# jaxsonpd/air_rs

Measured on AMD Instinct MI355X. Metric: IQ Msamples/s (decoded Mode-S msgs/s alongside), 2 MSPS i8 stream, higher is better.
Workload: dtype i8; 1 GPU; 2 MSPS i8 IQ, 1 GiB synthetic buffer per GPU, fused magnitude+preamble/DF17 gate+PPM+CRC-24; samples_per_gpu=536870912, bytes_per_gpu=1073741824, channels=1

## Files before the change

### air_rs_amd/csrc/adsb_kernels.hip

```cpp
#include <hip/hip_ext.h>
#include <utility>
#include <cstdlib>

#include "adsb_kernels.h"
#include "adsb_synth.h"

namespace adsbk {

typedef unsigned int u32x4 __attribute__((ext_vector_type(4)));
typedef unsigned short u16x2 __attribute__((ext_vector_type(2)));

__device__ __forceinline__ uint32_t pkmin(uint32_t a, uint32_t b)
{
    u16x2 r = __builtin_elementwise_min(__builtin_bit_cast(u16x2, a), __builtin_bit_cast(u16x2, b));
    return __builtin_bit_cast(uint32_t, r);
}
__device__ __forceinline__ uint32_t pkmax(uint32_t a, uint32_t b)
{
    u16x2 r = __builtin_elementwise_max(__builtin_bit_cast(u16x2, a), __builtin_bit_cast(u16x2, b));
    return __builtin_bit_cast(uint32_t, r);
}
typedef _Float16 f16x2 __attribute__((ext_vector_type(2)));
template <bool F16> __device__ __forceinline__ uint32_t pkmax3(uint32_t a, uint32_t b, uint32_t c)
{
    if (F16) {
        f16x2 r = __builtin_elementwise_maximum(
            __builtin_elementwise_maximum(__builtin_bit_cast(f16x2, a), __builtin_bit_cast(f16x2, b)),
            __builtin_bit_cast(f16x2, c));
        return __builtin_bit_cast(uint32_t, r);
    }
    return pkmax(pkmax(a, b), c);
}
template <bool F16> __device__ __forceinline__ uint32_t pkmin3(uint32_t a, uint32_t b, uint32_t c)
{
    if (F16) {
        f16x2 r = __builtin_elementwise_minimum(
            __builtin_elementwise_minimum(__builtin_bit_cast(f16x2, a), __builtin_bit_cast(f16x2, b)),
            __builtin_bit_cast(f16x2, c));
        return __builtin_bit_cast(uint32_t, r);
    }
    return pkmin(pkmin(a, b), c);
}

__device__ __forceinline__ void dot4x8_sacc(u32x4 v, int c, int n[8])
{
    const uint32_t a0 = v.x & 0xFFFFu, a1 = v.x & 0xFFFF0000u, a2 = v.y & 0xFFFFu, a3 = v.y & 0xFFFF0000u,
                   a4 = v.z & 0xFFFFu, a5 = v.z & 0xFFFF0000u, a6 = v.w & 0xFFFFu, a7 = v.w & 0xFFFF0000u;
    asm("v_dot4_i32_i8 %0, %8, %12, %20\n\t"
        "v_dot4_i32_i8 %1, %8, %13, %20\n\t"
        "v_dot4_i32_i8 %2, %9, %14, %20\n\t"
        "v_dot4_i32_i8 %3, %9, %15, %20\n\t"
        "v_dot4_i32_i8 %4, %10, %16, %20\n\t"
        "v_dot4_i32_i8 %5, %10, %17, %20\n\t"
        "v_dot4_i32_i8 %6, %11, %18, %20\n\t"
        "v_dot4_i32_i8 %7, %11, %19, %20\n\t"
        "s_nop 2"
        : "=&v"(n[0]), "=&v"(n[1]), "=&v"(n[2]), "=&v"(n[3]), "=&v"(n[4]), "=&v"(n[5]), "=&v"(n[6]), "=&v"(n[7])
        : "v"(v.x), "v"(v.y), "v"(v.z), "v"(v.w), "v"(a0), "v"(a1), "v"(a2), "v"(a3), "v"(a4), "v"(a5),
          "v"(a6), "v"(a7), "s"(c));
}

struct SynTable {
    uint32_t v[112];
};
constexpr SynTable make_syn()
{
    SynTable t{};
    uint32_t r = 1;
    for (int e = 0; e < 112; ++e) {
        t.v[111 - e] = r;
        r <<= 1;
        if (r & 0x1000000u) r ^= 0x1FFF409u;
    }
    return t;
}
__constant__ SynTable kSyn = make_syn();

template <int MAGMODE> __device__ __forceinline__ float mag_root_i8(int n_plus_2p23)
{
    float f = __builtin_bit_cast(float, n_plus_2p23) - 8388607.5f;
    float r = __builtin_amdgcn_sqrtf(f);
    if (MAGMODE == 2) r -= 0.5f;
    return r;
}

typedef float f32x2 __attribute__((ext_vector_type(2)));
template <int MAGMODE>
__device__ __forceinline__ void mags8_i8(u32x4 v, uint32_t &lo, uint32_t &hi)
{
    int n[8];
    dot4x8_sacc(v, 0x4B000000, n);
    float f[8];
#pragma unroll
    for (int k = 0; k < 8; k += 2) {
        f32x2 t = {__builtin_bit_cast(float, n[k]), __builtin_bit_cast(float, n[k + 1])};
        t = t - (f32x2){8388607.5f, 8388607.5f};
        f[k] = t.x;
        f[k + 1] = t.y;
    }
    float r[8];
#pragma unroll
    for (int k = 0; k < 8; ++k) {
        r[k] = __builtin_amdgcn_sqrtf(f[k]);
        if (MAGMODE == 2) r[k] -= 0.5f;
    }
    lo = __builtin_amdgcn_cvt_pk_u8_f32(r[0], 0, 0u);
    lo = __builtin_amdgcn_cvt_pk_u8_f32(r[1], 1, lo);
    lo = __builtin_amdgcn_cvt_pk_u8_f32(r[2], 2, lo);
    lo = __builtin_amdgcn_cvt_pk_u8_f32(r[3], 3, lo);
    hi = __builtin_amdgcn_cvt_pk_u8_f32(r[4], 0, 0u);
    hi = __builtin_amdgcn_cvt_pk_u8_f32(r[5], 1, hi);
    hi = __builtin_amdgcn_cvt_pk_u8_f32(r[6], 2, hi);
    hi = __builtin_amdgcn_cvt_pk_u8_f32(r[7], 3, hi);
}

__device__ __forceinline__ uint32_t mag_i16_fix(uint32_t r, uint32_t n)
{
    return r - ((__umul24(r, r) > n) ? 1u : 0u);
}
__device__ __forceinline__ uint32_t mag_i16(uint32_t iq)
{
    uint32_t n, r;
    asm("v_dot2_i32_i16 %0, %2, %2, 0\n\t"
        "s_nop 2\n\t"
        "v_cvt_f32_u32 %1, %0\n\t"
        "v_sqrt_f32 %1, %1\n\t"
        "s_nop 0\n\t"
        "v_cvt_rpi_i32_f32 %1, %1"
        : "=&v"(n), "=&v"(r)
        : "v"(iq));
    return mag_i16_fix(r, n);
}
__device__ __forceinline__ void mags4_i16(u32x4 v, uint32_t &lo, uint32_t &hi)
{
    uint32_t n0, n1, n2, n3, r0, r1, r2, r3;
    asm("v_dot2_i32_i16 %0, %8, %8, 0\n\t"
        "v_dot2_i32_i16 %1, %9, %9, 0\n\t"
        "v_dot2_i32_i16 %2, %10, %10, 0\n\t"
        "v_dot2_i32_i16 %3, %11, %11, 0\n\t"
        "s_nop 2\n\t"
        "v_cvt_f32_u32 %4, %0\n\t"
        "v_cvt_f32_u32 %5, %1\n\t"
        "v_cvt_f32_u32 %6, %2\n\t"
        "v_cvt_f32_u32 %7, %3\n\t"
        "v_sqrt_f32 %4, %4\n\t"
        "v_sqrt_f32 %5, %5\n\t"
        "v_sqrt_f32 %6, %6\n\t"
        "v_sqrt_f32 %7, %7\n\t"
        "v_cvt_rpi_i32_f32 %4, %4\n\t"
        "v_cvt_rpi_i32_f32 %5, %5\n\t"
        "v_cvt_rpi_i32_f32 %6, %6\n\t"
        "s_nop 0\n\t"
        "v_cvt_rpi_i32_f32 %7, %7\n\t"
        "s_nop 0"
        : "=&v"(n0), "=&v"(n1), "=&v"(n2), "=&v"(n3), "=&v"(r0), "=&v"(r1), "=&v"(r2), "=&v"(r3)
        : "v"(v.x), "v"(v.y), "v"(v.z), "v"(v.w));
    lo = __builtin_amdgcn_perm(mag_i16_fix(r1, n1), mag_i16_fix(r0, n0), 0x05040100u);
    hi = __builtin_amdgcn_perm(mag_i16_fix(r3, n3), mag_i16_fix(r2, n2), 0x05040100u);
}

__global__ void probe_cvt_kernel(uint32_t *out)
{
// ... 139 lines not shown
            "v_cmp_gt_u32_sdwa %7, %12, %12 src0_sel:BYTE_0 src1_sel:BYTE_1\n\t"
            "v_cmp_gt_u32_sdwa %8, %12, %12 src0_sel:BYTE_2 src1_sel:BYTE_3\n\t"
            "v_addc_co_u32_e64 %0, vcc, %0, %0, %1\n\t"
            "v_addc_co_u32_e64 %0, vcc, %0, %0, %2\n\t"
            "v_addc_co_u32_e64 %0, vcc, %0, %0, %3\n\t"
            "v_addc_co_u32_e64 %0, vcc, %0, %0, %4\n\t"
            "v_addc_co_u32_e64 %0, vcc, %0, %0, %5\n\t"
            "v_addc_co_u32_e64 %0, vcc, %0, %0, %6\n\t"
            "v_addc_co_u32_e64 %0, vcc, %0, %0, %7\n\t"
            "v_addc_co_u32_e64 %0, vcc, %0, %0, %8"
            : "+v"(byte), "=&s"(m0), "=&s"(m1), "=&s"(m2), "=&s"(m3), "=&s"(m4), "=&s"(m5), "=&s"(m6), "=&s"(m7)
            : "v"(w[0]), "v"(w[1]), "v"(w[2]), "v"(w[3])
            : "vcc");
    }
    return byte;
}

__device__ __forceinline__ uint32_t nsq_slice_byte(const uint32_t *img, const uint32_t off, const uint32_t l)
{
    const uint32_t half = off >= (uint32_t)kNsqHalf ? 1u : 0u;
    const uint32_t base = off - half * (uint32_t)kNsqHalf + 16u;
    const uint32_t e = base & 15u, par = e & 1u, sh = e >> 1;
    const uint32_t v = (base >> 4) + l;
    const uint32_t a1 = nsq_phys(16u * v) + par;
    constexpr uint32_t kChunksPerBlock = (1u << kNsqPadShift) / 16u;
    const uint32_t a2 = a1 + 15u + (((v & (kChunksPerBlock - 1u)) == kChunksPerBlock - 1u ? 4u : 0u) & (0u - par));
    uint32_t d[16];
#pragma unroll
    for (int j = 0; j < 15; ++j) d[j] = img[a1 + j];
    d[15] = img[a2];
    const uint32_t sel = half ? 0x07060302u : 0x05040100u;
    uint32_t w[8], r2[8];
#pragma unroll
    for (int j = 0; j < 8; ++j) {
        w[j] = __builtin_amdgcn_perm(d[2 * j + 1], d[2 * j], sel);
        const float fx = (float)(w[j] & 0xFFFFu) - ((float)kNsqBias - 0.5f);
        const uint32_t r = (uint32_t)__builtin_amdgcn_sqrtf(fx);
        r2[j] = __umul24(r, r) + (uint32_t)kNsqBias;
    }
    uint32_t chunk = 0;
    uint64_t m0, m1, m2, m3, m4, m5, m6, m7;
    asm("v_cmp_gt_u32_sdwa %1, %9, %17 src0_sel:DWORD src1_sel:WORD_1\n\t"
        "v_cmp_gt_u32_sdwa %2, %10, %18 src0_sel:DWORD src1_sel:WORD_1\n\t"
        "v_cmp_gt_u32_sdwa %3, %11, %19 src0_sel:DWORD src1_sel:WORD_1\n\t"
        "v_cmp_gt_u32_sdwa %4, %12, %20 src0_sel:DWORD src1_sel:WORD_1\n\t"
        "v_cmp_gt_u32_sdwa %5, %13, %21 src0_sel:DWORD src1_sel:WORD_1\n\t"
        "v_cmp_gt_u32_sdwa %6, %14, %22 src0_sel:DWORD src1_sel:WORD_1\n\t"
        "v_cmp_gt_u32_sdwa %7, %15, %23 src0_sel:DWORD src1_sel:WORD_1\n\t"
        "v_cmp_gt_u32_sdwa %8, %16, %24 src0_sel:DWORD src1_sel:WORD_1\n\t"
        "v_addc_co_u32_e64 %0, vcc, %0, %0, %1\n\t"
        "v_addc_co_u32_e64 %0, vcc, %0, %0, %2\n\t"
        "v_addc_co_u32_e64 %0, vcc, %0, %0, %3\n\t"
        "v_addc_co_u32_e64 %0, vcc, %0, %0, %4\n\t"
        "v_addc_co_u32_e64 %0, vcc, %0, %0, %5\n\t"
        "v_addc_co_u32_e64 %0, vcc, %0, %0, %6\n\t"
        "v_addc_co_u32_e64 %0, vcc, %0, %0, %7\n\t"
        "v_addc_co_u32_e64 %0, vcc, %0, %0, %8"
        : "+v"(chunk), "=&s"(m0), "=&s"(m1), "=&s"(m2), "=&s"(m3), "=&s"(m4), "=&s"(m5), "=&s"(m6), "=&s"(m7)
        : "v"(r2[0]), "v"(r2[1]), "v"(r2[2]), "v"(r2[3]), "v"(r2[4]), "v"(r2[5]), "v"(r2[6]), "v"(r2[7]),
          "v"(w[0]), "v"(w[1]), "v"(w[2]), "v"(w[3]), "v"(w[4]), "v"(w[5]), "v"(w[6]), "v"(w[7])
        : "vcc");
    const uint32_t next = (uint32_t)__builtin_amdgcn_update_dpp(0, (int)chunk, 0x101 , 0xF, 0xF, true);
    return (((chunk << 8) | next) >> (8u - sh)) & 0xFFu;
}

__device__ __forceinline__ bool count_candidate(const bool have, const uint32_t byte, const uint32_t l, const uint32_t lane)
{
    const uint32_t lb = l < 14 ? l : 13;
    uint32_t s = 0;
    const uint32_t *sy = kSyn.v + 8 * lb;
    const int sb = (int)(l < 14 ? byte : 0u);
#pragma unroll
    for (int k = 0; k < 8; ++k) s ^= sy[k] & (uint32_t)((sb << (24 + k)) >> 31);
    s = row16_xor(s);
    int found = -1;
    if (s != 0 && l < 11) {
#pragma unroll
        for (int k = 0; k < 8; ++k) found = (sy[k] == s) ? k : found;
    }
    const unsigned long long fm = __ballot(found >= 0);
    const uint32_t gbits = (uint32_t)(fm >> (lane & 48u)) & 0xFFFFu;
    return have && (s == 0 || gbits != 0);
}

struct TilePos {
    uint32_t ch;
    uint64_t sample0;
    uint32_t n_valid;
};
template <int TILE = kTile>
__device__ __forceinline__ TilePos tile_pos(const DemodArgs &p, uint32_t tile)
{
    TilePos t;
    t.ch = tile / p.tiles_per_channel;
    const uint32_t tch = tile - t.ch * p.tiles_per_channel;
    t.sample0 = (uint64_t)tch * TILE;
    const uint64_t left = (p.n_samples - kWindow) - t.sample0;
    t.n_valid = left < (uint64_t)TILE ? (uint32_t)left : (uint32_t)TILE;
    return t;
}

template <int BPS, int MAG = kMag>
__device__ __forceinline__ __amdgpu_buffer_rsrc_t tile_rsrc(const DemodArgs &p, const TilePos &t, bool live = true)
{
    const char *base = (const char *)p.iq + ((uint64_t)t.ch * p.channel_stride + t.sample0) * BPS;
    const uint64_t remain = (p.n_samples - t.sample0) * BPS;
    const uint32_t nrec = remain > (uint64_t)(MAG * BPS) ? (uint32_t)(MAG * BPS) : (uint32_t)remain;
    return __builtin_amdgcn_make_buffer_rsrc((void *)base, 0, live ? (int)nrec : 0, 0x00020000);
}

#ifndef ADSB_TILE_STAMPS
#define ADSB_TILE_STAMPS 0
#endif
#if ADSB_TILE_STAMPS
#define TSTAMP(k)                                                                                              \
    do {                                                                                                       \
        if ((tid & 63u) == 0 && (wave == 0 || wave == 3)) {                                                    \
            __builtin_amdgcn_sched_barrier(0);                                                                 \
            const unsigned long long now_ = __builtin_amdgcn_s_memtime();                                      \
            if ((k) >= 0) ts_seg[(k)] = (uint32_t)(now_ - ts_prev);                                            \
            ts_prev = now_;                                                                                    \
            __builtin_amdgcn_sched_barrier(0);                                                                 \
        }                                                                                                      \
    } while (0)
#else
#define TSTAMP(k) do { } while (0)
#endif

#ifndef ADSB_ABL_PHASES
#define ADSB_ABL_PHASES 3
#endif
#ifndef ADSB_ABL_NOCMP
#define ADSB_ABL_NOCMP 0
#endif
#ifndef ADSB_AB_KERNELS
#define ADSB_AB_KERNELS 0
#endif
bool ab_kernels_built() { return ADSB_AB_KERNELS != 0; }
#ifndef ADSB_PRIO
#define ADSB_PRIO 0
#endif
#ifndef ADSB_GATE_GROUP
#define ADSB_GATE_GROUP 1
#endif

template <int RUN, int NT>
__device__ __forceinline__ void gate_collect(uint32_t *candA, uint32_t *candB, uint16_t *list, uint32_t *count,
                                             const uint32_t tid, const uint32_t n_valid)
{
    constexpr int WPR = (RUN + 31) / 32;
    const uint32_t sa = tid * RUN, sb = (tid + NT) * RUN;
    const uint32_t va = n_valid > sa ? (n_valid - sa) : 0u, vb = n_valid > sb ? (n_valid - sb) : 0u;
    uint32_t words[2 * WPR];
    uint32_t nz = 0, c = 0;
#pragma unroll
    for (int k = 0; k < WPR; ++k) {
        words[k] = candA[k];
        words[WPR + k] = candB[k];
    }
    if (n_valid < (uint32_t)(2 * NT * RUN)) {
#pragma unroll
        for (int k = 0; k < WPR; ++k) {
            const uint32_t la = va > 32u * k ? va - 32u * k : 0u, lb = vb > 32u * k ? vb - 32u * k : 0u;
            words[k] &= la >= 32u ? 0xFFFFFFFFu : ((1u << la) - 1u);
            words[WPR + k] &= lb >= 32u ? 0xFFFFFFFFu : ((1u << lb) - 1u);
            candA[k] = words[k];
            candB[k] = words[WPR + k];
        }
    }
#pragma unroll
    for (int k = 0; k < 2 * WPR; ++k) {
        nz |= words[k];
        c += __builtin_popcount(words[k]);
    }
    if (nz) {
        uint32_t pos = atomicAdd(count, c);
#pragma unroll
        for (int k = 0; k < 2 * WPR; ++k) {
            uint32_t bits = words[k];
            const uint32_t base = (k < WPR ? sa : sb) + (k % WPR) * 32;
            while (bits) {
                const uint32_t b = __builtin_ctz(bits);
                bits &= bits - 1;
                if (pos < (uint32_t)kSparseCap) list[pos] = (uint16_t)(base + b);
                ++pos;
            }
        }
    }
}

struct NoHook {
    __device__ __forceinline__ void operator()() const {}
};

template <int ST, int GROUP, int RUN, int NT, int HOOK_AT = -1, class HOOK = NoHook, bool F16OK = (ST == ADSB_SAMPLE_I8), bool PAD = false>
__device__ __forceinline__ void gate_phase(const typename MagT<ST>::type *mag, uint32_t *cand, uint16_t *list,
                                           uint32_t *count, const uint32_t tid, const uint32_t n_valid,
                                           HOOK hook = HOOK())
{
    static_assert(RUN % GROUP == 0 && (RUN == 16 || RUN == 32 || RUN == 64), "steps are taken GROUP at a time; 1 or 2 bitmap words per run");
    constexpr int WPR = (RUN + 31) / 32;
    constexpr int SPG = 16 / (int)sizeof(typename MagT<ST>::type);
    uint32_t *candA = cand + WPR * tid, *candB = cand + WPR * (tid + NT);
#pragma unroll
    for (int k = 0; k < WPR; ++k) candA[k] = candB[k] = 0u;
    constexpr int kGran = (RUN + 26 + SPG - 1) / SPG + 1;
    static_assert(!PAD || (ST == ADSB_SAMPLE_I8 && RUN == 32 && (NT * RUN) % 256 == 0), "the padded image: u8 magnitudes, runs of 32 bytes");
    const u32x4 *ga = reinterpret_cast<const u32x4 *>(mag + mag_phys<PAD>(tid * RUN));
    const u32x4 *gb = reinterpret_cast<const u32x4 *>(mag + mag_phys<PAD>((tid + NT) * RUN));
    const uint32_t hop = PAD && (tid & 7u) == 7u ? 1u : 0u;
    const u32x4 *ga2 = ga + hop, *gb2 = gb + hop;
    uint32_t ra[kGran * 4], rb[kGran * 4];
    constexpr int kAhead = 48 / SPG;
#pragma unroll
    for (int g = 0; g < kAhead; ++g) {
        u32x4 a = (PAD && g >= 2) ? ga2[g] : ga[g], b = (PAD && g >= 2) ? gb2[g] : gb[g];
        ra[4 * g] = a.x; ra[4 * g + 1] = a.y; ra[4 * g + 2] = a.z; ra[4 * g + 3] = a.w;
        rb[4 * g] = b.x; rb[4 * g + 1] = b.y; rb[4 * g + 2] = b.z; rb[4 * g + 3] = b.w;
    }

    uint32_t N[RUN + 26], H2[RUN + 8], W3[RUN + 16], F[RUN + 9];
#pragma unroll
    for (int k = 0; k < 25; ++k) N[k] = pair_at<ST>(ra, rb, k);
#pragma unroll
    for (int j = 0; j < 7; ++j) H2[j] = pkmin(N[j], N[j + 2]);
#pragma unroll
    for (int j = 3; j < 13; ++j) W3[j] = pkmax3<F16OK>(N[j], N[j + 1], N[j + 2]);
#pragma unroll
    for (int j = 1; j < 8; ++j) F[j] = pkmax3<F16OK>(N[j], W3[j + 2], N[j + 5]);

#if ADSB_ABL_NOCMP
    uint32_t abl_acc = 0;
#endif
#pragma unroll
    for (int o0 = 0; o0 < RUN; o0 += GROUP) {
        if (o0 == HOOK_AT) hook();
        bool pa[GROUP], pb[GROUP];
        bool any = false;
#pragma unroll
        for (int gi = 0; gi < GROUP; ++gi) {
            const int o = o0 + gi;
            if (o % SPG == 0) {
                const int g = o / SPG + kAhead;
                if (g * SPG < RUN + 26) {
                    u32x4 a = (PAD && g >= 2) ? ga2[g] : ga[g], b = (PAD && g >= 2) ? gb2[g] : gb[g];
                    ra[4 * g] = a.x; ra[4 * g + 1] = a.y; ra[4 * g + 2] = a.z; ra[4 * g + 3] = a.w;
                    rb[4 * g] = b.x; rb[4 * g + 1] = b.y; rb[4 * g + 2] = b.z; rb[4 * g + 3] = b.w;
                }
            }
            N[o + 25] = pair_at<ST>(ra, rb, o + 25);
            W3[o + 13] = pkmax3<F16OK>(N[o + 13], N[o + 14], N[o + 15]);
            F[o + 8] = pkmax3<F16OK>(N[o + 8], W3[o + 10], N[o + 13]);
            const uint32_t lo = pkmax3<F16OK>(F[o + 1], F[o + 8], W3[o + 13]);
            H2[o + 7] = pkmin(N[o + 7], N[o + 9]);
            const uint32_t hi = pkmin(H2[o], H2[o + 7]);
#if ADSB_ABL_NOCMP
            abl_acc ^= hi ^ lo;
            pa[gi] = pb[gi] = false;
#else
            pa[gi] = (uint16_t)hi >= (uint16_t)lo;
            pb[gi] = (hi >> 16) >= (lo >> 16);
            any |= pa[gi] | pb[gi];
#endif
        }
        if (__builtin_expect(__builtin_amdgcn_ballot_w64(any) != 0, 0)) {
#pragma unroll
            for (int gi = 0; gi < GROUP; ++gi) {
                const int o = o0 + gi;
                if (GROUP == 1 || __builtin_amdgcn_ballot_w64(pa[gi] | pb[gi]) != 0) {
                    const uint32_t dh = pkmin3<F16OK>(pkmin3<F16OK>(N[o + 16], N[o + 19], N[o + 21]), N[o + 23], N[o + 24]);
                    const uint32_t dl = pkmax3<F16OK>(pkmax3<F16OK>(N[o + 17], N[o + 18], N[o + 20]), N[o + 22], N[o + 25]);
                    const bool da = (uint16_t)dh >= (uint16_t)dl;
                    const bool db = (dh >> 16) >= (dl >> 16);
                    uint32_t bit = 1u << (o & 31);
                    asm("" : "+v"(bit));
                    if (pa[gi] & da) atomicOr(candA + (o >> 5), bit);
                    if (pb[gi] & db) atomicOr(candB + (o >> 5), bit);
                }
            }
        }
    }
#if ADSB_ABL_NOCMP
    if (abl_acc == 0x12345678u) atomicOr(candA, 1u);
#endif
    gate_collect<RUN, NT>(candA, candB, list, count, tid, n_valid);
}

template <int BPS, int MAG = kMag>
__device__ __forceinline__ u32x4 tile_rsrc_words(const DemodArgs &p, const TilePos &t, bool live)
{
    const uint64_t base = (uint64_t)(uintptr_t)((const char *)p.iq + ((uint64_t)t.ch * p.channel_stride + t.sample0) * BPS);
    const uint64_t remain = (p.n_samples - t.sample0) * BPS;
    const uint32_t nrec = remain > (uint64_t)(MAG * BPS) ? (uint32_t)(MAG * BPS) : (uint32_t)remain;
    u32x4 w;
    w.x = __builtin_amdgcn_readfirstlane((uint32_t)base);
    w.y = __builtin_amdgcn_readfirstlane((uint32_t)(base >> 32) & 0xFFFFu);
    w.z = __builtin_amdgcn_readfirstlane(live ? nrec : 0u);
    w.w = 0x00020000u;
    return w;
}

#ifndef ADSB_LOAD_AUX
#define ADSB_LOAD_AUX 2
#endif
template <int ST> struct P1 {
    static constexpr int kSPL = ST == ADSB_SAMPLE_I8 ? 8 : 4;
    static constexpr int kIters = (TileCfg<ST>::kMagT + kThreads * kSPL - 1) / (kThreads * kSPL);
};

template <int ST>
__device__ __forceinline__ void issue_tile_loads(const DemodArgs &p, const TilePos &tp, bool live, uint32_t tid,
                                                 u32x4 (&raw)[P1<ST>::kIters])
{
    constexpr int BPS = (ST == ADSB_SAMPLE_I8) ? 2 : 4;
    __amdgpu_buffer_rsrc_t rsrc = tile_rsrc<BPS, TileCfg<ST>::kMagT>(p, tp, live);
    const uint32_t wave_s0 = __builtin_amdgcn_readfirstlane(tid & ~63u) * P1<ST>::kSPL;
#pragma unroll
    for (int it = 0; it < P1<ST>::kIters; ++it)
        if ((uint32_t)it * (kThreads * P1<ST>::kSPL) + wave_s0 < (uint32_t)TileCfg<ST>::kMagT)
            raw[it] = __builtin_amdgcn_raw_buffer_load_b128(rsrc, tid * 16, (uint32_t)it * (kThreads * 16), ADSB_LOAD_AUX);
}

template <int ST, int MAGMODE, bool PAD = false>
__device__ __forceinline__ bool magnitudes_to_lds(const u32x4 (&raw)[P1<ST>::kIters], typename MagT<ST>::type *mag, uint32_t tid)
{
    uint32_t mx = 0;
    const uint32_t wave_s0 = __builtin_amdgcn_readfirstlane(tid & ~63u) * P1<ST>::kSPL;
#pragma unroll
    for (int it = 0; it < P1<ST>::kIters; ++it) {
        if ((uint32_t)it * (kThreads * P1<ST>::kSPL) + wave_s0 < (uint32_t)TileCfg<ST>::kMagT) {
            const uint32_t s = (uint32_t)it * (kThreads * P1<ST>::kSPL) + tid * P1<ST>::kSPL;
            uint32_t lo, hi;
            if (ST == ADSB_SAMPLE_I8) mags8_i8<MAGMODE>(raw[it], lo, hi);
            else {
                mags4_i16(raw[it], lo, hi);
                mx = pkmax(mx, pkmax(lo, hi));
            }
            const uint32_t sp = PAD ? s + 16u * (tid >> 5) + (uint32_t)it * (16u * (kThreads * P1<ST>::kSPL / 256)) : s;
            if (s < (uint32_t)TileCfg<ST>::kMagT) *reinterpret_cast<uint2 *>(mag + sp) = make_uint2(lo, hi);
        }
    }
    return ST == ADSB_SAMPLE_I16 && __builtin_amdgcn_ballot_w64(((mx & 0xFFFFu) >= 0x7C00u) || ((mx >> 16) >= 0x7C00u)) != 0;
}

constexpr int kNsqIters = (kNsqLog + kThreads * 8 - 1) / (kThreads * 8);
constexpr int kNsqFull = kNsqLog / (kThreads * 8);
constexpr int kNsqTail = kNsqLog % (kThreads * 8);
static_assert(kNsqIters - kNsqFull <= 1 && kNsqTail % 8 == 0, "at most one partial sweep of whole lanes");

__device__ __forceinline__ void nsq_issue_loads(const DemodArgs &p, const TilePos &tp, uint32_t tid,
                                                u32x4 (&ra)[kNsqIters], u32x4 (&rb)[kNsqIters])
{
    __amdgpu_buffer_rsrc_t rsrc = tile_rsrc<2, kMag>(p, tp, true);
#pragma unroll
    for (int it = 0; it < kNsqFull; ++it) {
        ra[it] = __builtin_amdgcn_raw_buffer_load_b128(rsrc, tid * 16, (uint32_t)it * (kThreads * 16), ADSB_LOAD_AUX);
        rb[it] = __builtin_amdgcn_raw_buffer_load_b128(rsrc, tid * 16, (uint32_t)it * (kThreads * 16) + 2 * kNsqHalf, ADSB_LOAD_AUX);
    }
    if (kNsqTail && __builtin_amdgcn_readfirstlane(tid & ~63u) * 8 < (uint32_t)kNsqTail) {
        ra[kNsqFull] = __builtin_amdgcn_raw_buffer_load_b128(rsrc, tid * 16, (uint32_t)kNsqFull * (kThreads * 16), ADSB_LOAD_AUX);
        rb[kNsqFull] = __builtin_amdgcn_raw_buffer_load_b128(rsrc, tid * 16, (uint32_t)kNsqFull * (kThreads * 16) + 2 * kNsqHalf, ADSB_LOAD_AUX);
    }
}

__device__ __forceinline__ void nsq_pack16(u32x4 a, u32x4 b, uint32_t (&d)[8])
{
    const uint32_t a0 = a.x & 0xFFFFu, a1 = a.x & 0xFFFF0000u, a2 = a.y & 0xFFFFu, a3 = a.y & 0xFFFF0000u,
                   a4 = a.z & 0xFFFFu, a5 = a.z & 0xFFFF0000u, a6 = a.w & 0xFFFFu, a7 = a.w & 0xFFFF0000u;
    const uint32_t h0 = __builtin_amdgcn_perm(b.x, b.x, 0x010C000Cu), h1 = __builtin_amdgcn_perm(b.x, b.x, 0x030C020Cu),
                   h2 = __builtin_amdgcn_perm(b.y, b.y, 0x010C000Cu), h3 = __builtin_amdgcn_perm(b.y, b.y, 0x030C020Cu),
                   h4 = __builtin_amdgcn_perm(b.z, b.z, 0x010C000Cu), h5 = __builtin_amdgcn_perm(b.z, b.z, 0x030C020Cu),
                   h6 = __builtin_amdgcn_perm(b.w, b.w, 0x010C000Cu), h7 = __builtin_amdgcn_perm(b.w, b.w, 0x030C020Cu);
    const uint32_t bias2 = (uint32_t)kNsqBias * 0x00010001u;
    asm("v_dot4_i32_i8 %0, %8, %12, %28\n\t"
        "v_dot4_i32_i8 %1, %8, %13, %28\n\t"
        "v_dot4_i32_i8 %2, %9, %14, %28\n\t"
        "v_dot4_i32_i8 %3, %9, %15, %28\n\t"
        "v_dot4_i32_i8 %4, %10, %16, %28\n\t"
        "v_dot4_i32_i8 %5, %10, %17, %28\n\t"
        "v_dot4_i32_i8 %6, %11, %18, %28\n\t"
        "v_dot4_i32_i8 %7, %11, %19, %28\n\t"
        "v_dot2_i32_i16 %0, %20, %20, %0\n\t"
        "v_dot2_i32_i16 %1, %21, %21, %1\n\t"
        "v_dot2_i32_i16 %2, %22, %22, %2\n\t"
        "v_dot2_i32_i16 %3, %23, %23, %3\n\t"
        "v_dot2_i32_i16 %4, %24, %24, %4\n\t"
        "v_dot2_i32_i16 %5, %25, %25, %5\n\t"
        "v_dot2_i32_i16 %6, %26, %26, %6\n\t"
        "v_dot2_i32_i16 %7, %27, %27, %7\n\t"
        "s_nop 2"
        : "=&v"(d[0]), "=&v"(d[1]), "=&v"(d[2]), "=&v"(d[3]), "=&v"(d[4]), "=&v"(d[5]), "=&v"(d[6]), "=&v"(d[7])
        : "v"(a.x), "v"(a.y), "v"(a.z), "v"(a.w), "v"(a0), "v"(a1), "v"(a2), "v"(a3), "v"(a4), "v"(a5), "v"(a6), "v"(a7),
          "v"(h0), "v"(h1), "v"(h2), "v"(h3), "v"(h4), "v"(h5), "v"(h6), "v"(h7), "s"(bias2));
}

__device__ __forceinline__ bool nsq_image_to_lds(const u32x4 (&ra)[kNsqIters], const u32x4 (&rb)[kNsqIters], uint32_t *img, uint32_t tid)
{
    uint32_t lo = 0x7BFF7BFFu;
    const uint32_t q_t = tid * 8;
    uint32_t *dst = img + nsq_phys(q_t);
    auto sweep = [&](const int it, const bool store) {
        uint32_t d[8];
        nsq_pack16(ra[it], rb[it], d);
#pragma unroll
        for (int k = 0; k < 8; k += 2) lo = pkmin3<true>(lo, d[k], d[k + 1]);
        if (store) {
            u32x4 *w = reinterpret_cast<u32x4 *>(dst + nsq_phys(it * kThreads * 8));
            w[0] = u32x4{d[0], d[1], d[2], d[3]};
            w[1] = u32x4{d[4], d[5], d[6], d[7]};
        }
    };
#pragma unroll
    for (int it = 0; it < kNsqFull; ++it) sweep(it, true);
    if (kNsqTail && __builtin_amdgcn_readfirstlane(tid & ~63u) * 8 < (uint32_t)kNsqTail) sweep(kNsqFull, q_t < (uint32_t)kNsqTail);
    return __builtin_amdgcn_ballot_w64(((lo & 0xFFFFu) >= 0x7C00u) || ((lo >> 16) >= 0x7C00u)) != 0;
}

__device__ __forceinline__ uint32_t nsq_band(uint32_t x)
{
    const u16x2 v = __builtin_bit_cast(u16x2, x);
    return __builtin_bit_cast(uint32_t, (u16x2)(v + (v >> 3)));
}
__device__ __forceinline__ uint32_t nsq_root(uint32_t v)
{
    return (uint32_t)__builtin_amdgcn_sqrtf((float)v - ((float)kNsqBias - 0.5f));
}

#ifndef ADSB_NSQ_AHEAD
#define ADSB_NSQ_AHEAD 12
#endif
template <bool F16OK>
__device__ __forceinline__ void gate_phase_nsq(const uint32_t *img, uint32_t *cand, uint16_t *list, uint32_t *count,
                                               const uint32_t tid, const uint32_t n_valid)
{
    constexpr int RUN = kRun, NT = kThreads;
    uint32_t *candA = cand + tid, *candB = cand + (tid + NT);
    *candA = 0u;
    *candB = 0u;
    const u32x4 *g0 = reinterpret_cast<const u32x4 *>(img + nsq_phys(32 * tid));
    const u32x4 *g1 = reinterpret_cast<const u32x4 *>(img + nsq_phys(32 * tid + 32));
    constexpr int kGran = (RUN + 26 + 3) / 4;
    constexpr int kAhead = ADSB_NSQ_AHEAD;
    uint32_t N[kGran * 4];
    auto fetch = [&](int g) {
        const u32x4 x = g < 8 ? g0[g] : g1[g - 8];
        N[4 * g] = x.x; N[4 * g + 1] = x.y; N[4 * g + 2] = x.z; N[4 * g + 3] = x.w;
    };
#pragma unroll
    for (int g = 0; g < kAhead; ++g) fetch(g);
    uint32_t H2[RUN + 8], W3[RUN + 16], F[RUN + 9];
#pragma unroll
    for (int j = 0; j < 7; ++j) H2[j] = pkmin(N[j], N[j + 2]);
#pragma unroll
    for (int j = 3; j < 13; ++j) W3[j] = pkmax3<F16OK>(N[j], N[j + 1], N[j + 2]);
#pragma unroll
    for (int j = 1; j < 8; ++j) F[j] = pkmax3<F16OK>(N[j], W3[j + 2], N[j + 5]);

#pragma unroll
    for (int o = 0; o < RUN; ++o) {
        if (o % 4 == 0) {
            const int g = o / 4 + kAhead;
            if (g < kGran) fetch(g);
        }
        W3[o + 13] = pkmax3<F16OK>(N[o + 13], N[o + 14], N[o + 15]);
        F[o + 8] = pkmax3<F16OK>(N[o + 8], W3[o + 10], N[o + 13]);
        const uint32_t lo = pkmax3<F16OK>(F[o + 1], F[o + 8], W3[o + 13]);
        H2[o + 7] = pkmin(N[o + 7], N[o + 9]);
        const uint32_t hi = pkmin(H2[o], H2[o + 7]);
        const uint32_t t = nsq_band(hi);
        const bool pa = (uint16_t)t >= (uint16_t)lo;
        const bool pb = (t >> 16) >= (lo >> 16);
        if (__builtin_expect(__builtin_amdgcn_ballot_w64(pa | pb) != 0, 0)) {
            const uint32_t dh = pkmin3<F16OK>(pkmin3<F16OK>(N[o + 16], N[o + 19], N[o + 21]), N[o + 23], N[o + 24]);
            const uint32_t dl = pkmax3<F16OK>(pkmax3<F16OK>(N[o + 17], N[o + 18], N[o + 20]), N[o + 22], N[o + 25]);
            const uint32_t t2 = nsq_band(dh);
            bool sa = pa & ((uint16_t)t2 >= (uint16_t)dl);
            bool sb = pb & ((t2 >> 16) >= (dl >> 16));
            if (__builtin_amdgcn_ballot_w64(sa | sb) != 0) {
                const bool ea = ((uint16_t)hi >= (uint16_t)lo) & ((uint16_t)dh >= (uint16_t)dl);
                const bool eb = ((hi >> 16) >= (lo >> 16)) & ((dh >> 16) >= (dl >> 16));
                if (__builtin_expect(__builtin_amdgcn_ballot_w64((sa & !ea) | (sb & !eb)) != 0, 0)) {
                    const bool ra = nsq_root(hi & 0xFFFFu) >= nsq_root(lo & 0xFFFFu) && nsq_root(dh & 0xFFFFu) >= nsq_root(dl & 0xFFFFu);
                    const bool rb = nsq_root(hi >> 16) >= nsq_root(lo >> 16) && nsq_root(dh >> 16) >= nsq_root(dl >> 16);
                    sa = sa && (ea || ra);
                    sb = sb && (eb || rb);
                }
                uint32_t bit = 1u << o;
                asm("" : "+v"(bit));
                if (sa) atomicOr(candA, bit);
                if (sb) atomicOr(candB, bit);
            }
        }
    }
    gate_collect<RUN, NT>(candA, candB, list, count, tid, n_valid);
}

#ifndef ADSB_SCAN_WAVES
#define ADSB_SCAN_WAVES 4
#endif
#ifndef ADSB_REG_ABL
#define ADSB_REG_ABL 0
#endif
#ifndef ADSB_REG_WAVES
#define ADSB_REG_WAVES 5
#endif
template <int ST, int MAGMODE, int SCAN>
__device__ __forceinline__ void scan_tile(const DemodArgs &p, const uint32_t tile, const bool first, unsigned char *smem)
{
    typedef Lds<ST, SCAN> L;
    typedef TileCfg<ST> TC;
    typedef typename L::mag_t mag_t;
    constexpr bool NSQ = L::kNsq;
    static_assert(kThreads / 64 <= 4, "misc[4 + wave] must stay below misc[8]");

    mag_t *mag = reinterpret_cast<mag_t *>(smem);
    uint32_t *img = reinterpret_cast<uint32_t *>(smem);
    uint32_t *cand = reinterpret_cast<uint32_t *>(smem + L::kOffCand);
    uint16_t *list = reinterpret_cast<uint16_t *>(smem + L::kOffList);
    uint32_t *misc = reinterpret_cast<uint32_t *>(smem + L::kOffMisc);

    const uint32_t tid = threadIdx.x;
    const uint32_t lane = tid & 63, wave = tid >> 6;

#if ADSB_PRIO & 1
    __builtin_amdgcn_s_setprio(3);
#endif
    if (!NSQ && MAGMODE == 1) __builtin_amdgcn_s_setreg((1 | (0 << 6) | ((2 - 1) << 11)), 3);
#if ADSB_TILE_STAMPS
    unsigned long long ts_prev = 0;
    uint32_t ts_seg[9] = {0, 0, 0, 0, 0, 0, 0, 0, 0};
    ts_seg[7] = (uint32_t)__builtin_amdgcn_s_memrealtime();
    TSTAMP(-1);
    ts_seg[8] = (uint32_t)ts_prev;
#endif
    {
        const TilePos tp = tile_pos<TC::kTileT>(p, tile);
        const uint64_t sample0 = tp.sample0;
        const uint32_t n_valid = tp.n_valid;
        u32x4 raw[NSQ ? 1 : P1<ST>::kIters];
        u32x4 raw_a[NSQ ? kNsqIters : 1], raw_b[NSQ ? kNsqIters : 1];
        if constexpr (NSQ) nsq_issue_loads(p, tp, tid, raw_a, raw_b);
        else issue_tile_loads<ST>(p, tp, true, tid, raw);
#if ADSB_PRIO & 1
        __builtin_amdgcn_s_setprio(0);
#endif
        TSTAMP(0);
        if (tid == 0 && first) {
            p.hdr->retry = 0;
            if (p.count_groups) {
                p.hdr->flags = 0;
                if (p.hdr_pub) p.hdr_pub[2] = 0;
            }
        }
        if (tid == 0) {
            misc[8] = 0;
            misc[12] = 0;
        }
#if ADSB_TILE_STAMPS
        asm volatile("s_waitcnt vmcnt(0)" ::: "memory");
        TSTAMP(6);
#endif
        bool wave_big;
        if constexpr (NSQ) wave_big = nsq_image_to_lds(raw_a, raw_b, img, tid);
        else wave_big = magnitudes_to_lds<ST, MAGMODE, MagPad<ST, SCAN>::on>(raw, mag, tid);
        if ((NSQ || ST == ADSB_SAMPLE_I16) && lane == 0) misc[4 + wave] = wave_big ? 1u : 0u;
        TSTAMP(1);
        __syncthreads();
        TSTAMP(2);
#if ADSB_ABL_PHASES < 2
        if (smem[tid * 64] == 0xFD && smem[tid * 64 + 1] == 0xFE && n_valid == 7) misc[12] = 1;
#else

        if constexpr (NSQ || ST == ADSB_SAMPLE_I16) {
            uint32_t any_big = 0;
#pragma unroll
            for (int w = 0; w < kThreads / 64; ++w) any_big |= misc[4 + w];
            const bool big = any_big != 0;
            if constexpr (NSQ) {
                if (!big) gate_phase_nsq<true>(img, cand, list, &misc[12], tid, n_valid);
                else gate_phase_nsq<false>(img, cand, list, &misc[12], tid, n_valid);
            } else {
                if (!big) gate_phase<ST, ADSB_GATE_GROUP, TC::kRunT, kThreads, -1, NoHook, true>(mag, cand, list, &misc[12], tid, n_valid);
                else gate_phase<ST, ADSB_GATE_GROUP, TC::kRunT, kThreads, -1, NoHook, false>(mag, cand, list, &misc[12], tid, n_valid);
            }
        } else {
            gate_phase<ST, ADSB_GATE_GROUP, TC::kRunT, kThreads, -1, NoHook, (ST == ADSB_SAMPLE_I8), MagPad<ST, SCAN>::on>(mag, cand, list, &misc[12], tid, n_valid);
        }
#endif
        TSTAMP(3);
        __syncthreads();
        TSTAMP(4);

#if ADSB_PRIO & 2
        __builtin_amdgcn_s_setprio(2);
#endif
        uint32_t total = misc[12];
#if ADSB_ABL_PHASES < 3
        if (total != 0x7FFFFFFFu) total = 0;
#endif
        const bool dense = total > (uint32_t)kSparseCap;
        constexpr int kBitsPerWord = TC::kRunT < 32 ? TC::kRunT : 32;
        u32x4 cw = {0, 0, 0, 0};
        uint32_t cnt = 0, my_first = 0;
        if (dense) {
            if (4 * tid < (uint32_t)(TC::kTileT / kBitsPerWord)) cw = reinterpret_cast<const u32x4 *>(cand)[tid];
            cnt = __builtin_popcount(cw.x) + __builtin_popcount(cw.y) + __builtin_popcount(cw.z) +
                  __builtin_popcount(cw.w);
            uint32_t incl = cnt;
#pragma unroll
            for (int d = 1; d < 64; d <<= 1) {
                uint32_t t = __shfl_up(incl, d, 64);
                if ((int)lane >= d) incl += t;
            }
            if (lane == 63) misc[wave] = incl;
            __syncthreads();
            uint32_t wbase = 0;
            total = 0;
#pragma unroll
            for (int w = 0; w < kThreads / 64; ++w) {
                uint32_t t = misc[w];
                wbase += (w < (int)wave) ? t : 0u;
                total += t;
            }
            my_first = wbase + incl - cnt;
        }

        const bool simple = !dense && total <= kQuota;
        const uint64_t abs0 = sample0 + p.offset_base;
        uint32_t base_slot = tile * kQuota;
        const uint32_t g = tid >> 4, l = tid & 15;
        auto slice_one = [&](uint32_t off) {
            if constexpr (NSQ) return nsq_slice_byte(img, off, l);
            else return slice_byte<ST, MagPad<ST, SCAN>::on>(mag, off, l < 14 ? l : 13);
        };
        auto slice_round = [&](uint32_t slot0, uint32_t ncl) {
            for (uint32_t r = 0; r < ncl; r += kThreads / 16) {
                if (r + 4 * wave >= ncl) break;
                const uint32_t ci = r + g;
                const bool have = ci < ncl;
                const uint32_t off = have ? list[ci] : 0u;
                const uint32_t byte = slice_one(off);
                if (have) {
                    unsigned char *rec = reinterpret_cast<unsigned char *>(p.slots + (size_t)slot0 + ci);
                    const uint64_t o64 = abs0 + off;
                    if (l < 14) rec[8 + l] = (unsigned char)byte;
                    else reinterpret_cast<uint32_t *>(rec)[l - 14] = l == 14 ? (uint32_t)o64 : (uint32_t)(o64 >> 32);
                }
            }
        };
        if (simple) {
            slice_round(base_slot, total);
        } else {
            if (tid == 0) {
                const unsigned long long b64 = atomicAdd(&p.hdr->alloc, (unsigned long long)total);
                misc[9] = (!p.pool_off && b64 + total <= (unsigned long long)p.cap_slots) ? p.pool_first + (uint32_t)b64 : kNoBase;
            }
            __syncthreads();
            base_slot = misc[9];
            for (uint32_t chunk = 0; chunk < total; chunk += kListCap) {
                if (dense && cnt) {
                    uint32_t idx = my_first;
                    const uint32_t words[4] = {cw.x, cw.y, cw.z, cw.w};
#pragma unroll
                    for (int k = 0; k < 4; ++k) {
                        uint32_t bits = words[k];
                        while (bits) {
                            const uint32_t b = __builtin_ctz(bits);
                            bits &= bits - 1;
                            if (idx >= chunk && idx < chunk + kListCap)
                                list[idx - chunk] = (uint16_t)((4 * tid + k) * kBitsPerWord + b);
                            ++idx;
                        }
                    }
                }
                __syncthreads();
                const uint32_t ncl = (total - chunk) < (uint32_t)kListCap ? (total - chunk) : (uint32_t)kListCap;
                if (base_slot != kNoBase) {
                    slice_round(base_slot + chunk, ncl);
                } else {
                    for (uint32_t r = 0; r < ncl; r += kThreads / 16) {
                        if (r + 4 * wave >= ncl) break;
                        const uint32_t ci = r + g;
                        const bool have = ci < ncl;
                        const uint32_t off = have ? list[ci] : 0u;
                        const bool valid = count_candidate(have, slice_one(off), l, lane);
                        if (valid && l == 0) atomicAdd(&misc[8], 1u);
                    }
                }
                __syncthreads();
            }
        }
        TSTAMP(5);
#if ADSB_TILE_STAMPS
        if ((tid & 63u) == 0 && (wave == 0 || wave == 3)) {
            uint32_t *dst = reinterpret_cast<uint32_t *>(p.stamps) + (size_t)tile * 16 + (wave ? 8 : 0);
#pragma unroll
            for (int k = 0; k < 8; ++k) dst[k] = ts_seg[k];
            if (wave) dst[6] = ts_seg[8];
        }
#endif
        if (tid == 0) {
            Seg e;
            e.base = base_slot;
            e.cand = total;
            e.valid = misc[8];
            e.decoded = base_slot == kNoBase ? 1u : 0u;
            p.seg[tile] = e;
        }
    }
    if (!NSQ && MAGMODE == 1) __builtin_amdgcn_s_setreg((1 | (0 << 6) | ((2 - 1) << 11)), 0);
}

#ifndef ADSB_XCD_MAP
#define ADSB_XCD_MAP 1
#endif
__device__ __forceinline__ uint32_t tile_of_workgroup(uint32_t b, uint32_t n)
{
#if ADSB_XCD_MAP
    const uint32_t q = n >> 3, r = n & 7u, x = b & 7u, j = b >> 3;
    return x * q + (x < r ? x : r) + j;
#else
    (void)n;
    return b;
#endif
}

template <int ST, int MAGMODE, int SCAN>
__global__ __launch_bounds__(kThreads, (ST == ADSB_SAMPLE_I8 && SCAN == kScanRoot) ? 8 : ADSB_SCAN_WAVES) void demod_tiles(DemodArgs p)
{
    __shared__ __attribute__((aligned(16))) unsigned char smem[Lds<ST, SCAN>::kTotal];
    scan_tile<ST, MAGMODE, SCAN>(p, p.tile_first + tile_of_workgroup(blockIdx.x, p.tile_count), blockIdx.x == 0, smem);
}

struct CrcTable {
    uint32_t v[256];
};
constexpr CrcTable make_crc_table()
{
    CrcTable t{};
    for (uint32_t i = 0; i < 256; ++i) {
        uint32_t r = i << 16;
        for (int k = 0; k < 8; ++k) {
            r <<= 1;
            if (r & 0x1000000u) r ^= 0x1FFF409u;
        }
        t.v[i] = r & 0xFFFFFFu;
    }
    return t;
}
__constant__ CrcTable kCrcTab = make_crc_table();
struct SynSorted {
    uint32_t v[128];
};
constexpr SynSorted make_syn_sorted()
{
    SynSorted t{};
    SynTable sy = make_syn();
    for (int j = 0; j < 128; ++j) t.v[j] = j < 88 ? ((sy.v[j] << 7) | (uint32_t)j) : 0xFFFFFFFFu;
    for (int i = 1; i < 128; ++i) {
        uint32_t x = t.v[i];
        int k = i - 1;
        while (k >= 0 && t.v[k] > x) {
            t.v[k + 1] = t.v[k];
            --k;
        }
        t.v[k + 1] = x;
    }
    return t;
}
__constant__ SynSorted kSynSorted = make_syn_sorted();

constexpr int kFinTiles = 32;
constexpr int kFinThreads = 256;
constexpr int kFinFan = 64;
constexpr int kFinFlat = 1024;
constexpr uint32_t kLbReady = 1u;
constexpr uint32_t kLbSpinLimit = 1u << 21;

__device__ __forceinline__ bool finish_record(uint32_t (&w)[6], const bool have, const uint32_t *crc_tab, const uint32_t *syn_sorted)
{
    uint32_t crc = 0;
#pragma unroll
    for (int i = 0; i < 11; ++i) {
        const uint32_t b = (w[2 + (i >> 2)] >> (8 * (i & 3))) & 0xFFu;
        crc = ((crc << 8) ^ crc_tab[((crc >> 16) ^ b) & 0xFFu]) & 0xFFFFFFu;
    }
    const uint32_t rx = ((w[4] >> 24) << 16) | ((w[5] & 0xFFu) << 8) | ((w[5] >> 8) & 0xFFu);
    const uint32_t sm = crc ^ rx;
    uint32_t pos = 0;
#pragma unroll
    for (int step = 64; step >= 1; step >>= 1)
        pos += ((syn_sorted[pos + step - 1] >> 7) < sm) ? (uint32_t)step : 0u;
    const uint32_t hit = syn_sorted[pos];
    const bool found = sm != 0 && (hit >> 7) == sm;
    const bool valid = have && (sm == 0 || found);
    const bool fix = valid && sm != 0;
    const uint32_t fixed = fix ? (hit & 0x7Fu) : 0xFFu;
    const uint32_t status = valid ? (sm == 0 ? 0u : 1u) : 0xFFu;
    const uint32_t bi = 8u + ((hit & 0x7Fu) >> 3);
    const uint32_t flip = fix ? ((0x80u >> (hit & 7u)) << (8u * (bi & 3u))) : 0u;
    const uint32_t wi = bi >> 2;
    w[2] ^= wi == 2 ? flip : 0u;
    w[3] ^= wi == 3 ? flip : 0u;
    w[4] ^= wi == 4 ? flip : 0u;
    w[5] = (w[5] & 0xFFFFu) | (status << 16) | (fixed << 24);
    return valid;
}


template <int N> __device__ __forceinline__ uint32_t row_ror(uint32_t v)
{
// ... 1342 lines not shown
```

Before: 2.696 million Msamples/s.

## Append gate candidates to list inline with wave-aggregated LDS atomic

Removes the post-scan gate_collect pass that popcounted the bitmap words and appended candidates. Each hit now appends its offset directly to the sparse list, using a ballot, mbcnt rank and a single ds_add_rtn per wave, while still setting the bitmap bit. Lane masks from ballots are reused instead of recomputing them. Because hits are rare, the per-tile collect cost is replaced by occasional inline appends. List order changes, and the cap clamp now overwrites the last slot instead of dropping entries. The wave index is also made uniform with readfirstlane.

```diff
diff --git a/air_rs_amd/csrc/adsb_kernels.hip b/air_rs_amd/csrc/adsb_kernels.hip
--- a/air_rs_amd/csrc/adsb_kernels.hip
+++ b/air_rs_amd/csrc/adsb_kernels.hip
@@ -490,6 +490,34 @@
     }
 }
 
+template <int RUN, int NT>
+__device__ __forceinline__ void gate_record(bool a, bool b, const int o, uint32_t *candA, uint32_t *candB,
+                                            uint16_t *list, uint32_t *count, const uint32_t tid, const uint32_t n_valid)
+{
+    const uint32_t oa = tid * RUN + (uint32_t)o, ob = (tid + NT) * RUN + (uint32_t)o;
+    const uint32_t lds_count = (uint32_t)(size_t)(__attribute__((address_space(3))) uint32_t *)count;
+    a = a && oa < n_valid;
+    b = b && ob < n_valid;
+    auto append = [&](uint32_t off) {
+        const uint64_t m = __builtin_amdgcn_ballot_w64(true);
+        const uint32_t rank = __builtin_amdgcn_mbcnt_hi((uint32_t)(m >> 32), __builtin_amdgcn_mbcnt_lo((uint32_t)m, 0u));
+        uint32_t base = (uint32_t)__builtin_popcountll(m);
+        if (rank == 0)
+            asm volatile("ds_add_rtn_u32 %0, %1, %0\n\ts_waitcnt lgkmcnt(0)" : "+v"(base) : "v"(lds_count) : "memory");
+        uint32_t pos = __builtin_amdgcn_readfirstlane(base) + rank;
+        pos = pos < (uint32_t)kListCap - 1u ? pos : (uint32_t)kListCap - 1u;
+        list[pos] = (uint16_t)off;
+    };
+    if (a) {
+        append(oa);
+        atomicOr(candA + (o >> 5), 1u << (o & 31));
+    }
+    if (b) {
+        append(ob);
+        atomicOr(candB + (o >> 5), 1u << (o & 31));
+    }
+}
+
 struct NoHook {
     __device__ __forceinline__ void operator()() const {}
 };
@@ -537,7 +565,8 @@
     for (int o0 = 0; o0 < RUN; o0 += GROUP) {
         if (o0 == HOOK_AT) hook();
         bool pa[GROUP], pb[GROUP];
-        bool any = false;
+        uint64_t ma[GROUP], mb[GROUP];
+        uint64_t any = 0;
 #pragma unroll
         for (int gi = 0; gi < GROUP; ++gi) {
             const int o = o0 + gi;
@@ -558,25 +587,25 @@
 #if ADSB_ABL_NOCMP
             abl_acc ^= hi ^ lo;
             pa[gi] = pb[gi] = false;
+            ma[gi] = mb[gi] = 0;
 #else
             pa[gi] = (uint16_t)hi >= (uint16_t)lo;
             pb[gi] = (hi >> 16) >= (lo >> 16);
-            any |= pa[gi] | pb[gi];
-#endif
-        }
-        if (__builtin_expect(__builtin_amdgcn_ballot_w64(any) != 0, 0)) {
+            ma[gi] = __builtin_amdgcn_ballot_w64(pa[gi]);
+            mb[gi] = __builtin_amdgcn_ballot_w64(pb[gi]);
+            any |= ma[gi] | mb[gi];
+#endif
+        }
+        if (__builtin_expect(any != 0, 0)) {
 #pragma unroll
             for (int gi = 0; gi < GROUP; ++gi) {
                 const int o = o0 + gi;
-                if (GROUP == 1 || __builtin_amdgcn_ballot_w64(pa[gi] | pb[gi]) != 0) {
+                if (GROUP == 1 || (ma[gi] | mb[gi]) != 0) {
                     const uint32_t dh = pkmin3<F16OK>(pkmin3<F16OK>(N[o + 16], N[o + 19], N[o + 21]), N[o + 23], N[o + 24]);
                     const uint32_t dl = pkmax3<F16OK>(pkmax3<F16OK>(N[o + 17], N[o + 18], N[o + 20]), N[o + 22], N[o + 25]);
-                    const bool da = (uint16_t)dh >= (uint16_t)dl;
-                    const bool db = (dh >> 16) >= (dl >> 16);
-                    uint32_t bit = 1u << (o & 31);
-                    asm("" : "+v"(bit));
-                    if (pa[gi] & da) atomicOr(candA + (o >> 5), bit);
-                    if (pb[gi] & db) atomicOr(candB + (o >> 5), bit);
+                    const bool da = (uint16_t)dh >= (uint16_t)dl, db = (dh >> 16) >= (dl >> 16);
+                    const uint64_t both = (ma[gi] & __builtin_amdgcn_ballot_w64(da)) | (mb[gi] & __builtin_amdgcn_ballot_w64(db));
+                    if (__builtin_expect(both != 0, 0)) gate_record<RUN, NT>(pa[gi] & da, pb[gi] & db, o, candA, candB, list, count, tid, n_valid);
                 }
             }
         }
@@ -584,7 +613,6 @@
 #if ADSB_ABL_NOCMP
     if (abl_acc == 0x12345678u) atomicOr(candA, 1u);
 #endif
-    gate_collect<RUN, NT>(candA, candB, list, count, tid, n_valid);
 }
 
 template <int BPS, int MAG = kMag>
@@ -821,7 +849,7 @@
     uint32_t *misc = reinterpret_cast<uint32_t *>(smem + L::kOffMisc);
 
     const uint32_t tid = threadIdx.x;
-    const uint32_t lane = tid & 63, wave = tid >> 6;
+    const uint32_t lane = tid & 63, wave = __builtin_amdgcn_readfirstlane(tid >> 6);
 
 #if ADSB_PRIO & 1
     __builtin_amdgcn_s_setprio(3);
```

After: 2.728 million Msamples/s (median of 6 runs). 1.2% higher.

## Use wave-level ballot compaction in gate_collect and DPP-gathered slot writes

Applied to the files above, without the earlier changes.

gate_collect now builds the candidate list with wave ballots: one LDS atomic per wave per round and mbcnt-based positions, in place of a per-thread atomicAdd followed by a serial ctz loop. The slice writer gathers the 16 per-lane bytes into one lane through DPP row shuffles, and that lane writes the whole record as two wide stores instead of 16 scattered byte and word stores. Uniform values are also moved to scalar registers with readfirstlane. The costs are extra ballot and DPP instructions, inline asm for the LDS atomic, and clamped out-of-range list reads.

```diff
diff --git a/air_rs_amd/csrc/adsb_kernels.hip b/air_rs_amd/csrc/adsb_kernels.hip
--- a/air_rs_amd/csrc/adsb_kernels.hip
+++ b/air_rs_amd/csrc/adsb_kernels.hip
@@ -8,6 +8,7 @@
 namespace adsbk {
 
 typedef unsigned int u32x4 __attribute__((ext_vector_type(4)));
+typedef unsigned int u32x4_a8 __attribute__((ext_vector_type(4), aligned(8)));
 typedef unsigned short u16x2 __attribute__((ext_vector_type(2)));
 
 __device__ __forceinline__ uint32_t pkmin(uint32_t a, uint32_t b)
@@ -453,7 +454,6 @@
     const uint32_t sa = tid * RUN, sb = (tid + NT) * RUN;
     const uint32_t va = n_valid > sa ? (n_valid - sa) : 0u, vb = n_valid > sb ? (n_valid - sb) : 0u;
     uint32_t words[2 * WPR];
-    uint32_t nz = 0, c = 0;
 #pragma unroll
     for (int k = 0; k < WPR; ++k) {
         words[k] = candA[k];
@@ -469,25 +469,39 @@
             candB[k] = words[WPR + k];
         }
     }
+    uint64_t m[2 * WPR];
+    uint64_t any = 0;
 #pragma unroll
     for (int k = 0; k < 2 * WPR; ++k) {
-        nz |= words[k];
-        c += __builtin_popcount(words[k]);
-    }
-    if (nz) {
-        uint32_t pos = atomicAdd(count, c);
+        m[k] = __builtin_amdgcn_ballot_w64(words[k] != 0u);
+        any |= m[k];
+    }
+    if (!any) return;
+    const uint32_t lane = __lane_id();
+    const uint32_t count_lds = (uint32_t)(uintptr_t)count;
+    do {
+        uint32_t n = 0;
+#pragma unroll
+        for (int k = 0; k < 2 * WPR; ++k) n += (uint32_t)__builtin_popcountll(m[k]);
+        uint32_t got = 0;
+        if (lane == 0) asm volatile("ds_add_rtn_u32 %0, %1, %2\n\ts_waitcnt lgkmcnt(0)" : "=v"(got) : "v"(count_lds), "v"(n) : "memory");
+        uint32_t pos0 = __builtin_amdgcn_readfirstlane(got);
+        any = 0;
 #pragma unroll
         for (int k = 0; k < 2 * WPR; ++k) {
-            uint32_t bits = words[k];
-            const uint32_t base = (k < WPR ? sa : sb) + (k % WPR) * 32;
-            while (bits) {
-                const uint32_t b = __builtin_ctz(bits);
-                bits &= bits - 1;
-                if (pos < (uint32_t)kSparseCap) list[pos] = (uint16_t)(base + b);
-                ++pos;
-            }
-        }
-    }
+            if (m[k]) {
+                if (words[k]) {
+                    const uint32_t pos = pos0 + __builtin_amdgcn_mbcnt_hi((uint32_t)(m[k] >> 32), __builtin_amdgcn_mbcnt_lo((uint32_t)m[k], 0u));
+                    const uint32_t base = (k < WPR ? sa : sb) + (k % WPR) * 32;
+                    list[min(pos, (uint32_t)kSparseCap)] = (uint16_t)(base + __builtin_ctz(words[k]));
+                }
+                words[k] &= words[k] - 1u;
+                pos0 += (uint32_t)__builtin_popcountll(m[k]);
+                m[k] = __builtin_amdgcn_ballot_w64(words[k] != 0u);
+                any |= m[k];
+            }
+        }
+    } while (any);
 }
 
 struct NoHook {
@@ -895,7 +909,7 @@
 #if ADSB_PRIO & 2
         __builtin_amdgcn_s_setprio(2);
 #endif
-        uint32_t total = misc[12];
+        uint32_t total = __builtin_amdgcn_readfirstlane(misc[12]);
 #if ADSB_ABL_PHASES < 3
         if (total != 0x7FFFFFFFu) total = 0;
 #endif
@@ -929,23 +943,31 @@
         const bool simple = !dense && total <= kQuota;
         const uint64_t abs0 = sample0 + p.offset_base;
         uint32_t base_slot = tile * kQuota;
-        const uint32_t g = tid >> 4, l = tid & 15;
+        uint32_t tid3 = tid;
+        asm volatile("" : "+v"(tid3));
+        const uint32_t g = tid3 >> 4, l = tid3 & 15;
         auto slice_one = [&](uint32_t off) {
             if constexpr (NSQ) return nsq_slice_byte(img, off, l);
             else return slice_byte<ST, MagPad<ST, SCAN>::on>(mag, off, l < 14 ? l : 13);
         };
+        const uint32_t wave_u = __builtin_amdgcn_readfirstlane(tid3 >> 6), row = (tid3 >> 4) & 3u;
+        const uint32_t byte_sh = 8u * (tid3 & 3u);
         auto slice_round = [&](uint32_t slot0, uint32_t ncl) {
-            for (uint32_t r = 0; r < ncl; r += kThreads / 16) {
-                if (r + 4 * wave >= ncl) break;
-                const uint32_t ci = r + g;
-                const bool have = ci < ncl;
-                const uint32_t off = have ? list[ci] : 0u;
-                const uint32_t byte = slice_one(off);
-                if (have) {
-                    unsigned char *rec = reinterpret_cast<unsigned char *>(p.slots + (size_t)slot0 + ci);
+            unsigned char *const rec0 = reinterpret_cast<unsigned char *>(p.slots + slot0);
+            for (uint32_t r = 4u * wave_u; r < ncl; r += kThreads / 16) {
+                const uint32_t ci = r + row;
+                const uint32_t off = min((uint32_t)list[ci], (uint32_t)(TC::kTileT - 1));
+                uint32_t v = slice_one(off) << byte_sh;
+                v |= ADSB_DPP(v, 0xB1);
+                v |= ADSB_DPP(v, 0x4E);
+                const uint32_t d1 = ADSB_DPP(v, 0x104);
+                const uint32_t d2 = ADSB_DPP(v, 0x108);
+                const uint32_t d3 = ADSB_DPP(v, 0x10C);
+                if (l == 0 && ci < ncl) {
                     const uint64_t o64 = abs0 + off;
-                    if (l < 14) rec[8 + l] = (unsigned char)byte;
-                    else reinterpret_cast<uint32_t *>(rec)[l - 14] = l == 14 ? (uint32_t)o64 : (uint32_t)(o64 >> 32);
+                    unsigned char *rec = rec0 + ci * (uint32_t)sizeof(adsb_frame);
+                    *reinterpret_cast<u32x4_a8 *>(rec) = (u32x4_a8){(uint32_t)o64, (uint32_t)(o64 >> 32), v, d1};
+                    *reinterpret_cast<uint2 *>(rec + 16) = make_uint2(d2, d3);
                 }
             }
         };
@@ -957,7 +979,7 @@
                 misc[9] = (!p.pool_off && b64 + total <= (unsigned long long)p.cap_slots) ? p.pool_first + (uint32_t)b64 : kNoBase;
             }
             __syncthreads();
-            base_slot = misc[9];
+            base_slot = __builtin_amdgcn_readfirstlane(misc[9]);
             for (uint32_t chunk = 0; chunk < total; chunk += kListCap) {
                 if (dense && cnt) {
                     uint32_t idx = my_first;
```

After: 2.647 million Msamples/s before, 2.670 million Msamples/s after (median of 6 runs). About the same (+0.9%).
